# AlessioSam/LADiff

Hardware: AMD Instinct MI355X
Metric: motions/sec (196-frame, 50-step DDIM, bs128) (higher is better)
Workload: dtype f16x3+f32; 1 GPU; headline:ddim50_cfg7.5_b128_f196_c263_humanml3d; prompts_per_gpu=128, global_batch=128, frames=196, scheduler=ddim, denoising_steps=50, parallelism=dp1, loop=persistent pipeline kernel (16-row blocks x 86)

## Files before the change

### ladiff_amd/build.py

```python
import os
import subprocess
import sys
from concurrent.futures import ThreadPoolExecutor

HERE = os.path.dirname(os.path.abspath(__file__))
CSRC = os.path.join(HERE, "csrc")
OBJ = os.path.join(HERE, "csrc", "build")
LIB = os.path.join(HERE, "libladiff_hip.so")
SOURCES = ["gemm.hip", "gemm_big.hip", "gemm_kr.hip", "gemm_rowln.hip", "rowops.hip", "attention.hip", "qkv_attn.hip", "systolic.hip", "linear_ca.hip", "dec_cross.hip", "dec_mlp.hip", "dec_qkv_attn.hip", "feats2joints.hip", "denoiser.hip", "decoder.hip", "encoder.hip", "clip.hip", "evaluator.hip", "api.hip"]
FLAGS = ["--offload-arch=gfx950", "-O3", "-std=c++17", "-fPIC", "-fvisibility=hidden", "-Wall", "-Wno-unused-function"]


def _hipcc():
    for c in (os.environ.get("HIPCC"), "/opt/rocm/bin/hipcc", "hipcc"):
        if c and (os.path.isabs(c) and os.path.exists(c) or not os.path.isabs(c)):
            return c
    raise RuntimeError("hipcc not found")


def _stale(target, deps):
    if not os.path.exists(target):
        return True
    t = os.path.getmtime(target)
    return any(os.path.getmtime(d) > t for d in deps)


def stamps_lib(level=1):
    return LIB.replace(".so", "_stamps.so" if int(level) == 1 else f"_stamps{int(level)}.so")


def diag_lib():
    return LIB.replace(".so", "_diag.so")


def build(force=False, verbose=False, stamps=False, tag=None, defines=(), only=None):
    obj, lib, flags = OBJ, LIB, list(FLAGS)
    if tag:
        obj, lib = OBJ + "_" + tag, LIB.replace(".so", f"_{tag}.so")
        flags += ["-D" + d for d in defines]
    if stamps:
        lvl = os.environ.get("LADIFF_STAMPS_LEVEL", "1")
        obj, lib = OBJ + "_stamps" + (lvl if lvl != "1" else ""), stamps_lib(lvl)
        flags.append("-DLADIFF_STAMPS=" + lvl)
    os.makedirs(obj, exist_ok=True)
    headers = [os.path.join(CSRC, f) for f in os.listdir(CSRC) if f.endswith(".h")]
    headers += [os.path.join(os.path.dirname(HERE), "include", h) for h in ("ladiff_hip.h", "ladiff_hip_debug.h")]
    hipcc = _hipcc()
    jobs = []
    objdir = {src: (obj if only is None or src in only else OBJ) for src in SOURCES}
    for src in SOURCES:
        s = os.path.join(CSRC, src)
        o = os.path.join(objdir[src], src.replace(".hip", ".o"))
        if objdir[src] == obj and (force or _stale(o, [s] + headers)):
            jobs.append([hipcc, *flags, "-c", s, "-o", o])

    def run(cmd):
        if verbose:
            print(" ".join(cmd), flush=True)
        r = subprocess.run(cmd, capture_output=True, text=True)
        if r.returncode != 0:
            raise RuntimeError(f"hipcc failed: {' '.join(cmd)}\n{r.stdout}\n{r.stderr}")
        return r.stderr
# ... 27 lines not shown
```

### ladiff_amd/csrc/api.hip

```cpp
#include <algorithm>
#include <cstdlib>
#include <atomic>
#include <cstdio>
#include <cstdlib>
#include <cstring>
#include <vector>

#include "model.h"
#include "../../include/ladiff_hip_debug.h"

using namespace ladiff;

namespace {

inline hipStream_t S(ladiff_stream_t s) { return reinterpret_cast<hipStream_t>(s); }

template <class W>
bool load_weights(W& dst, const float* const* ptrs) {
    constexpr int n = sizeof(W) / sizeof(const float*);
    if (ptrs == nullptr) return false;
    for (int i = 0; i < n; ++i)
        if (ptrs[i] == nullptr) return false;
    std::memcpy(&dst, ptrs, sizeof(W));
    return true;
// ... 307 lines not shown
    int mr16 = 1, nb16 = 0, mr32 = 2, nb32 = 0;
    std::vector<unsigned char> p16, p32;
    if (!cfg) {
        sys_pack_blocks(B, T, 1, h_counts, masked, false, plan, plan_mr, plan_nb);
        return;
    }
    sys_pack_blocks(B, T, 2, h_counts, masked, true, p32, &mr32, &nb32);
    int want = loop_mode == 2 ? 1 : (loop_mode == 3 ? 2 : 0);
    if (want != 2) sys_pack_blocks(B, T, 1, h_counts, masked, true, p16, &mr16, &nb16);
    if (want == 0) {
        const double c16 = f16x3 ? 2.45 : 5.05, c32 = f16x3 ? 5.3 : 12.1, lat16 = f16x3 ? 172.0 : 310.0, lat32 = f16x3 ? 282.0 : 525.0;
        const double e16 = mr16 == 1 ? std::max(lat16, nb16 * c16) : 1e30, e32 = std::max(lat32, nb32 * c32);
        want = e16 < e32 ? 1 : 2;
    }
    if (want == 1 && mr16 == 1) { plan.swap(p16); *plan_mr = 1; *plan_nb = nb16; }
    else { plan.swap(p32); *plan_mr = 2; *plan_nb = nb32; }
}

extern "C" {

int ladiff_reverse_plan(int B, int T, const int32_t* h_counts, int masked, int loop_mode, int f16x3, int cfg, int* rows_per_block, int* n_blocks) {
    LADIFF_CHECK_ARG(B >= 1 && T >= 1 && T <= LADIFF_MAX_LATENTS && loop_mode >= 1 && loop_mode <= 3 && rows_per_block && n_blocks);
    if (!cfg && masked && h_counts == nullptr) return LADIFF_ERR_UNSUPPORTED;
    std::vector<unsigned char> plan;
    int mr = 2, nb = 0;
    choose_plan(B, T, h_counts, masked != 0, loop_mode, f16x3 != 0, plan, &mr, &nb, cfg != 0);
    *rows_per_block = 16 * mr; *n_blocks = nb;
    return 0;
}

int ladiff_debug_set_stage_waves(int waves_per_simd) {
    LADIFF_CHECK_ARG(waves_per_simd == 1 || waves_per_simd == 2);
    g_waves16 = waves_per_simd;
    return 0;
}

int ladiff_debug_set_handoff(int tagged) {
    LADIFF_CHECK_ARG(tagged == 0 || tagged == 1);
    g_handoff = tagged;
    return 0;
}

int ladiff_debug_set_mlp_variant(int v) {
#ifdef LADIFF_STAMPS
    LADIFF_CHECK_ARG((v >= 0 && v <= 3) || (v >= 11 && v <= 17) || (v >= 21 && v <= 26));
#else
    LADIFF_CHECK_ARG(v >= 0 && v <= 3);
#endif
    g_mlp_variant = v;
    return 0;
}

int ladiff_debug_set_decoder_fusion(int on) {
    LADIFF_CHECK_ARG(on >= 0 && on <= 126 && (on & 3) != 3 && (on & 48) != 48);
    g_dec_out_cross = (on & 64) ? 0 : 1;
    g_dec_fused_mlp = on & 3;
    g_dec_small_rows_path = (on & 4) ? 0 : 1;
    g_dec_final_split = (on & 8) ? 0 : 1;
    g_dec_fused_attn = (on & 16) ? 0 : (on & 32) ? 2 : 1;
    return 0;
}

int ladiff_debug_set_stage_plan(int v) {
    LADIFF_CHECK_ARG(v >= 0 && v <= 1);
    g_stage_plan = v;
    return 0;
}

int ladiff_debug_set_poll_pause(int mask, int len) {
    LADIFF_CHECK_ARG(mask >= 0 && mask <= 255 && len >= 0 && len <= 64);
    g_poll_pause = mask | (len << 8);
    return 0;
}

int ladiff_debug_set_pacing(int eighths, int mask) {
    if (eighths == -1) { g_pace = -1; return 0; }
    LADIFF_CHECK_ARG(eighths >= 0 && eighths <= 8 && mask >= 0 && mask <= 255);
    g_pace = eighths | (mask << 8);
    return 0;
}

int ladiff_debug_set_stage_delay(int mask, int len) {
    LADIFF_CHECK_ARG(mask >= -1 && mask <= 255 && len >= 0 && len <= 64);
    g_stage_delay = mask < 0 ? -1 : (mask | (len << 8));
    return 0;
}

int ladiff_debug_set_loop_thresholds(int look_ahead_from, int small_upto) {
    LADIFF_CHECK_ARG(look_ahead_from >= -1 && small_upto >= -1);
    g_look_ahead_from = look_ahead_from;
    g_small_upto = small_upto;
    return 0;
}

int ladiff_debug_set_graph_epoch_rule(int on) {
    LADIFF_CHECK_ARG(on == 0 || on == 1);
    g_graph_epoch_rule = on;
    return 0;
}

int ladiff_debug_graph_instantiations(void) { return g_graph_instantiations.load(); }

int ladiff_debug_set_xcd_local(int on) {
    LADIFF_CHECK_ARG(on >= 0 && on <= 2);
    g_xcd_local = on;
    return 0;
}
// ... 351 lines not shown
    (void)C;
    return dec_ws_floats(B, (size_t)B * F, T) * sizeof(float);
}

int ladiff_vae_decode(const float* const* w, const float* const* w_split, const float* z, const int32_t* lengths,
                      const int32_t* counts, int B, int F, int T, int C, float* feats, void* ws, size_t ws_bytes,
                      ladiff_stream_t stream) {
    DecoderW W, WS;
    LADIFF_CHECK_ARG(load_weights(W, w) && z && lengths && feats && ws && B >= 0);
    if (w_split != nullptr) LADIFF_CHECK_ARG(load_weights(WS, w_split));
    return vae_decode(W, w_split ? &WS : nullptr, z, lengths, counts, nullptr, 0, B, F, T, C, feats, (float*)ws, ws_bytes / sizeof(float),
                      S(stream));
}

namespace {
struct DecodeGraph {
    hipGraphExec_t exec = nullptr;
    hipStream_t cap = nullptr;
    int cap_dev = -1;
    const void* key_ptrs[7] = {nullptr};
    uint64_t epoch = 0;
    int key_ints[6] = {0};
    uint64_t key_hash = 0, key_gen = 0;
};
}

int ladiff_decoder_graph_create(void** graph) {
    LADIFF_CHECK_ARG(graph);
    *graph = new DecodeGraph();
    return 0;
}
int ladiff_decoder_graph_destroy(void* graph) {
    DecodeGraph* g = reinterpret_cast<DecodeGraph*>(graph);
    if (g == nullptr) return 0;
    (void)hipDeviceSynchronize();
    if (g->exec) (void)hipGraphExecDestroy(g->exec);
    if (g->cap) (void)hipStreamDestroy(g->cap);
    delete g;
    return 0;
}

int ladiff_vae_decode_graphed(void* graph, const float* const* w, const float* const* w_split, uint64_t weights_generation, const float* z,
                              const int32_t* lengths, const int32_t* counts, const int32_t* row_off, int total_rows, int B, int F, int T,
                              int C, float* feats, void* ws, size_t ws_bytes, ladiff_stream_t stream) {
    DecodeGraph* dg = reinterpret_cast<DecodeGraph*>(graph);
    DecoderW W, WS;
    LADIFF_CHECK_ARG(dg && load_weights(W, w) && z && lengths && feats && ws && B >= 0 && stream != nullptr);
    if (w_split != nullptr) LADIFF_CHECK_ARG(load_weights(WS, w_split));
    hipStream_t s = S(stream);
    const void* kp[7] = {z, lengths, counts, row_off, feats, ws, stream};
    const int ki[6] = {B, F, T, C, total_rows, w_split ? 1 : 0};
    uint64_t h = hash_ptrs(w, DEC_NPARAMS, 1469598103934665603ull);
    if (w_split) h = hash_ptrs(w_split, DEC_NPARAMS, h ^ 0x9e3779b97f4a7c15ull);
    h ^= (uint64_t)(g_dec_fused_mlp + 4 * g_dec_small_rows_path + 8 * g_dec_final_split + 16 * g_mlp_variant + 4096 * g_dec_fused_attn) * 0x100000001b3ull;
    const bool same = dg->exec && std::memcmp(kp, dg->key_ptrs, sizeof(kp)) == 0 && std::memcmp(ki, dg->key_ints, sizeof(ki)) == 0 &&
                      h == dg->key_hash && weights_generation == dg->key_gen &&
                      (dg->epoch == g_graph_epoch.load() || g_graph_epoch_rule.load() == 0);
    if (!same) {
        if (dg->exec) { LADIFF_HIP(hipStreamSynchronize(s)); (void)hipGraphExecDestroy(dg->exec); dg->exec = nullptr; }
        LADIFF_TRY(dec_mlp_prepare());
        LADIFF_TRY(dec_qkv_attn_prepare());
        LADIFF_TRY(dec_cross_prepare());
        hipGraph_t gr = nullptr;
        LADIFF_TRY(capture_stream(&dg->cap, &dg->cap_dev));
        const hipStream_t cs = dg->cap;
        LADIFF_HIP(hipStreamBeginCapture(cs, hipStreamCaptureModeThreadLocal));
        int rc = 0;
        if (row_off != nullptr) {
            rc = launch_zero_fill(feats, (size_t)B * F * C, cs);
        }
        if (rc == 0) rc = vae_decode(W, w_split ? &WS : nullptr, z, lengths, counts, row_off, total_rows, B, F, T, C, feats, (float*)ws,
                                     ws_bytes / sizeof(float), cs);
        const hipError_t ec = hipStreamEndCapture(cs, &gr);
        if (rc != 0) { if (gr) (void)hipGraphDestroy(gr); return rc; }
        LADIFF_HIP(ec);
        const hipError_t ei = hipGraphInstantiate(&dg->exec, gr, nullptr, nullptr, 0);
        ++g_graph_instantiations;
        (void)hipGraphDestroy(gr);
        LADIFF_HIP(ei);
        std::memcpy(dg->key_ptrs, kp, sizeof(kp));
        std::memcpy(dg->key_ints, ki, sizeof(ki));
        dg->key_hash = h; dg->key_gen = weights_generation;
        dg->epoch = ++g_graph_epoch;
    }
    LADIFF_HIP(hipGraphLaunch(dg->exec, s));
    return 0;
}

int ladiff_vae_decode_ragged(const float* const* w, const float* const* w_split, const float* z, const int32_t* lengths,
                             const int32_t* counts, const int32_t* row_off, int total_rows, int B, int F, int T, int C, float* feats,
                             void* ws, size_t ws_bytes, ladiff_stream_t stream) {
    DecoderW W, WS;
    LADIFF_CHECK_ARG(load_weights(W, w) && z && lengths && row_off && feats && ws && B >= 0 && total_rows >= 0);
    if (w_split != nullptr) LADIFF_CHECK_ARG(load_weights(WS, w_split));
    LADIFF_HIP(hipMemsetAsync(feats, 0, (size_t)B * F * C * sizeof(float), S(stream)));
    return vae_decode(W, w_split ? &WS : nullptr, z, lengths, counts, row_off, total_rows, B, F, T, C, feats, (float*)ws,
                      ws_bytes / sizeof(float), S(stream));
}

}
```

### ladiff_amd/csrc/decoder.hip

```cpp
#include "model.h"
#ifdef LADIFF_STAMPS
#include <cstdlib>
#endif

namespace ladiff {

#ifdef LADIFF_STAMPS
#define DEC_CUT() do { if (dec_cut >= 0 && ++dec_launched >= dec_cut) return 0; } while (0)
#else
#define DEC_CUT() do { } while (0)
#endif

constexpr int DEC_SMALL_ROWS = 4096;
std::atomic<int> g_dec_out_cross{1};
std::atomic<int> g_dec_fused_attn{1};
std::atomic<int> g_dec_final_split{1};
std::atomic<int> g_dec_small_rows_path{1};
std::atomic<int> g_dec_fused_mlp{1};

static GemmArgs lin(const float* A, int lda, const float* W, const float* bias, float* Y, int ldy, int M, int N, int K,
                    int act = ACT_NONE) {
    GemmArgs g;
    g.A = A; g.lda = lda; g.W = W; g.ldw = K; g.bias = bias; g.Y = Y; g.ldy = ldy; g.M = M; g.N = N; g.K = K; g.act = act;
    return g;
}

size_t dec_ws_floats(int B, size_t rows, int T) {
    return rows * (16 * D + 3 * D + D + FF) + (rows + 63) / 64 * 64 + (size_t)NL * ((size_t)T * B * 2 * D + dec_cross_ws_floats(B, T)) +
           (size_t)LADIFF_MAX_FRAMES * (2 * D + 3 * D);
}

int vae_decode(const DecoderW& w, const DecoderW* wsp, const float* z, const int32_t* lengths, const int32_t* counts,
               const int32_t* row_off, int R, int B, int F, int T, int C, float* feats, float* ws, size_t ws_floats, hipStream_t s) {
    if (F < 1 || F > LADIFF_MAX_FRAMES || T < 1 || T > LADIFF_MAX_LATENTS || C < 1) return LADIFF_ERR_SHAPE;
    const bool ragged = row_off != nullptr;
    if (ragged && (R < 0 || (size_t)R > (size_t)B * F)) return LADIFF_ERR_SHAPE;
    const int M = ragged ? R : B * F;
    if (ws_floats < dec_ws_floats(B, (size_t)M, T)) return LADIFF_ERR_WORKSPACE;
    if (M == 0) return 0;
#ifdef LADIFF_STAMPS
    const char* dec_cut_env = getenv("LADIFF_DEC_CUT");
    const int dec_cut = dec_cut_env ? atoi(dec_cut_env) : -1;
    int dec_launched = 0;
    if (dec_cut == 0) return 0;
#endif
    const bool sp = wsp != nullptr;
    const size_t MD = (size_t)M * D;
    float* P[4]; float* SK[NSKIP]; float* Ps[4]; float* SKs[NSKIP];
    float* p = ws;
    for (int i = 0; i < 4; ++i) { P[i] = p; p += MD; }
    for (int i = 0; i < NSKIP; ++i) { SK[i] = p; p += MD; }
    for (int i = 0; i < 4; ++i) { Ps[i] = sp ? p : nullptr; p += MD; }
    for (int i = 0; i < NSKIP; ++i) { SKs[i] = sp ? p : nullptr; p += MD; }
    float* qkv = p; p += 3 * MD;
    float* att = p; p += MD;
    float* hid = p; p += (size_t)M * FF;
    float* kv = p; p += (size_t)NL * T * B * 2 * D;
    float* guws = p; p += (size_t)NL * dec_cross_ws_floats(B, T);
    int32_t* row_out = reinterpret_cast<int32_t*>(p); p += ((size_t)M + 63) / 64 * 64;
    float* pex = p; p += (size_t)LADIFF_MAX_FRAMES * D;
    float* pexs = p; p += (size_t)LADIFF_MAX_FRAMES * D;
    float* qkv0 = p;
    const size_t kv_l = (size_t)T * B * 2 * D, gu_l = dec_cross_ws_floats(B, T);

    {
        GemmArgs g[NL];
        DecCrossPrepBatch pb;
        for (int l = 0; l < NL; ++l) {
            const DecLayerW& L = w.layer[l];
            g[l] = lin(z, D, L.cross_attn.in_w + (size_t)D * D, L.cross_attn.in_b + D, kv + l * kv_l, 2 * D, T * B, 2 * D, D);
// ... 26 lines not shown
        g.split = 1;
        LADIFF_TRY(launch_gemm(g, s));
        if (n2)
            return launch_reduce_rows(dst, 1, M, nullptr, nullptr, RED_LN, n1.g, n1.b, nullptr, 0, nullptr, nullptr, 1, 1, 0,
                                      0, dst, dsts, s, nullptr, n2->g, n2->b);
        return launch_reduce_rows(dst, 1, M, nullptr, nullptr, RED_LN, n1.g, n1.b, nullptr, 0, nullptr, nullptr, 1, 1, 0, 0,
                                  dst, dsts, s);
    };

    if (ragged) { LADIFF_TRY(launch_broadcast_pe_ragged(w.query_pe, row_off, B, F, F, P[0], Ps[0], row_out, s)); DEC_CUT(); }
    else { LADIFF_TRY(launch_broadcast_pe(w.query_pe, B, F, P[0], Ps[0], s)); DEC_CUT(); }
    const float* cur = P[0]; const float* curs = Ps[0];
    for (int l = 0; l < NL; ++l) {
        const DecLayerW& L = w.layer[l];
        const DecLayerW& Ls = sp ? wsp->layer[l] : w.layer[l];
        const bool is_in = l < NSKIP, is_out = l > NSKIP, last = l == NL - 1;
        if (is_out) {
            const LinearW& sk = w.skip[l - NSKIP - 1];
            if (small) {
                RowLnArgs g;
                g.A = curs; g.lda = D; g.A2 = SKs[NL - 1 - l]; g.lda2 = D; g.K1 = D; g.W = wsp->skip[l - NSKIP - 1].w; g.ldw = 2 * D; g.bias = sk.b;
                g.Y = P[3]; g.Ys = Ps[3]; g.ldy = D; g.M = M; g.K = 2 * D;
                LADIFF_TRY(launch_gemm_rowln(g, s)); DEC_CUT();
            } else {
            GemmArgs g = lin(sp ? curs : cur, D, sp ? wsp->skip[l - NSKIP - 1].w : sk.w, sk.b, P[3], D, M, D, 2 * D);
            g.A2 = sp ? SKs[NL - 1 - l] : SK[NL - 1 - l]; g.lda2 = D; g.K1 = D;
            g.split = sp ? 1 : 0; g.Ys = Ps[3];
            LADIFF_TRY(launch_gemm(g, s)); DEC_CUT();
            }
            cur = P[3]; curs = Ps[3];
        }
        const bool shared = l == 0;
        if (shared) {
            LADIFF_TRY(launch_broadcast_pe(w.query_pe, 1, F, pex, sp ? pexs : nullptr, s)); DEC_CUT();
            if (small) { LADIFF_TRY(krs(pexs, D, Ls.self_attn.in_w, L.self_attn.in_b, qkv0, nullptr, 3 * D, 3 * D, ACT_NONE, nullptr, F)); DEC_CUT(); }
            else {
            GemmArgs g = lin(sp ? pexs : pex, D, Ls.self_attn.in_w, L.self_attn.in_b, qkv0, 3 * D, F, 3 * D, D);
            g.split = sp ? 1 : 0;
            LADIFF_TRY(launch_gemm(g, s)); DEC_CUT();
            }
        } else if (fused_attn) {
        } else if (small) {
            LADIFF_TRY(krs(curs, D, Ls.self_attn.in_w, L.self_attn.in_b, qkv, nullptr, 3 * D, 3 * D, ACT_NONE, nullptr, M)); DEC_CUT();
        } else {
            GemmArgs g = lin(sp ? curs : cur, D, Ls.self_attn.in_w, L.self_attn.in_b, qkv, 3 * D, M, 3 * D, D);
            g.split = sp ? 1 : 0;
            LADIFF_TRY(launch_gemm(g, s)); DEC_CUT();
        }
        const float* qkv_l = shared ? qkv0 : qkv;
        if (fused_attn && !shared) { LADIFF_TRY(launch_dec_qkv_attn(curs, Ls.self_attn.in_w, L.self_attn.in_b, lengths, row_off, att, B, F, 1, s)); DEC_CUT(); }
        else if (sp) { LADIFF_TRY(launch_self_attention_split(qkv_l, lengths, nullptr, att, B, F, H, 0, 1, s, row_off, shared)); DEC_CUT(); }
        else { LADIFF_TRY(launch_decoder_self_attention(qkv_l, lengths, nullptr, att, B, F, 0, s, row_off, shared)); DEC_CUT(); }
        const NormW* n1_late = nullptr;
        if (sp && !small && g_dec_out_cross) {
            LADIFF_TRY(launch_decoder_out_cross(att, cur, Ls.self_attn.out_w, L.self_attn.out_b, L.norm1.g, L.norm1.b, L.cross_attn.out_b,
                                                L.norm2.g, L.norm2.b, counts, B, F, T, guws + l * gu_l, P[2], Ps[2], s, row_off)); DEC_CUT();
        } else {
        if (sp) {
            if (small) { LADIFF_TRY(krs(att, D, Ls.self_attn.out_w, L.self_attn.out_b, P[1], nullptr, D, D, ACT_NONE, cur, M)); DEC_CUT(); }
            else {
            GemmArgs g = lin(att, D, Ls.self_attn.out_w, L.self_attn.out_b, P[1], D, M, D, D);
            g.res = cur; g.ldres = D; g.split = 1;
            LADIFF_TRY(launch_gemm(g, s)); DEC_CUT();
            }
            n1_late = &L.norm1;
        } else {
            LADIFF_TRY(gemm_ln(att, D, L.self_attn.out_w, Ls.self_attn.out_w, L.self_attn.out_b, cur, L.norm1, nullptr, P[1], nullptr)); DEC_CUT();
        }
        LADIFF_TRY(launch_decoder_cross_apply(P[1], L.cross_attn.out_b, L.norm2.g, L.norm2.b, counts, B, F, T, guws + l * gu_l, P[2],
                                              Ps[2], s, row_off, n1_late ? n1_late->g : nullptr, n1_late ? n1_late->b : nullptr)); DEC_CUT();
        }
        float* dst = is_in ? SK[l] : P[0];
        float* dsts = is_in ? SKs[l] : Ps[0];
        if (sp && g_dec_fused_mlp && (M >= dec_mlp_min_rows() || g_dec_fused_mlp == 2)) {
            LADIFF_TRY(launch_dec_mlp(Ps[2], P[2], Ls.lin1.w, L.lin1.b, Ls.lin2.w, L.lin2.b, L.norm3.g, L.norm3.b,
                                      last ? w.norm.g : nullptr, last ? w.norm.b : nullptr, dst, dsts, M, s)); DEC_CUT();
        } else if (small) {
            LADIFF_TRY(krs(Ps[2], D, Ls.lin1.w, L.lin1.b, nullptr, hid, FF, FF, ACT_GELU, nullptr, M)); DEC_CUT();
            LADIFF_TRY(krs(hid, FF, Ls.lin2.w, nullptr, qkv, nullptr, D, D, ACT_NONE, nullptr, M)); DEC_CUT();
            LADIFF_TRY(launch_reduce_rows(qkv, 4, M, L.lin2.b, P[2], RED_LN, L.norm3.g, L.norm3.b, nullptr, 0, nullptr, nullptr, 1, 1, 0, 0,
                                          dst, dsts, s, nullptr, last ? w.norm.g : nullptr, last ? w.norm.b : nullptr));
        } else {
            GemmArgs g = lin(sp ? Ps[2] : P[2], D, Ls.lin1.w, L.lin1.b, sp ? nullptr : hid, FF, M, FF, D, ACT_GELU);
            g.split = sp ? 1 : 0; if (sp) g.Ys = hid;
            LADIFF_TRY(launch_gemm(g, s)); DEC_CUT();
            LADIFF_TRY(gemm_ln(hid, FF, L.lin2.w, Ls.lin2.w, L.lin2.b, P[2], L.norm3, last ? &w.norm : nullptr, dst, dsts)); DEC_CUT();
        }
        cur = dst; curs = dsts;
    }
    if (sp && M >= DEC_SMALL_ROWS && g_dec_final_split) {
        const int Np = (C + 127) / 128 * 128;
        if ((size_t)Np > (size_t)FF || (size_t)Np * (D + 1) > 3 * MD) return LADIFF_ERR_SHAPE;
        float* wpad = qkv; float* bpad = qkv + (size_t)Np * D;
        LADIFF_TRY(launch_pad_rows(wsp->final_layer.w, w.final_layer.b, wpad, bpad, C, Np, s)); DEC_CUT();
        GemmArgs g = lin(curs, D, wpad, bpad, hid, Np, M, Np, D);
        g.split = 1;
        LADIFF_TRY(launch_gemm(g, s)); DEC_CUT();
        return launch_scatter_feats(hid, Np, C, M, F, ragged ? nullptr : lengths, ragged ? row_out : nullptr, feats, s);
    }
    GemmArgs g = lin(cur, D, w.final_layer.w, w.final_layer.b, feats, C, M, C, D);
    if (ragged) g.row_map = row_out;
    else { g.row_len = lengths; g.rows_per_item = F; }
    return launch_gemm(g, s);
}

}
```

### ladiff_amd/csrc/model.h

```cpp
#pragma once
#include <atomic>
#include "gemm.h"
#include "gemm_kr.h"
#include "kernels.h"
#include "weights.h"

namespace ladiff {

constexpr int DEN_OFF_CA_MOD = 0;
constexpr int DEN_OFF_FFN_MOD = 2 * D;
constexpr int DEN_OFF_TIME_KV = 4 * D;
constexpr int DEN_LAYER_STRIDE = 6 * D;
constexpr int DEN_STEP_STRIDE = NL * DEN_LAYER_STRIDE;

size_t den_tables_floats(int n_steps);
size_t den_text_cache_floats(int B2, int n_steps, int ntxt = 1);
size_t den_text_ws_floats(int B2, int n_steps, int ntxt = 1);
size_t den_forward_ws_floats(int B2, int T);
int denoiser_time_tables(const DenoiserW& w, const float* sinus, int n, float* tables, float* ws, size_t ws_floats, hipStream_t s);
int denoiser_text_cache(const DenoiserW& w, const float* text, int B2, const float* tables, int n_steps, float* cache,
                        float* ws, size_t ws_floats, hipStream_t s, int ntxt = 1);
int denoiser_forward(const DenoiserW& w, const DenoiserW* w_split, const float* tables, const int32_t* d_step,
                     const float* cache, int n_steps, const float* sample, int Bs, int dup, int T, const int32_t* counts, float* eps, float* ws,
                     size_t ws_floats, hipStream_t s, int b_lo = 0, int b_n = -1, int loop_mode = 0, int ntxt = 1,
                     const int32_t* d_base = nullptr);
const float* den_cache_tkv(const float* cache, int B2, int ntxt);
const float* den_cache_ctab(const float* cache, int B2, int ntxt);
int denoiser_text_static(const DenoiserW& w, const float* text, int B2, float* cache, float* ws, size_t ws_floats, hipStream_t s);
int denoiser_ctab(const DenoiserW& w, const float* tables_lo, int n, float* cache, int B2, float* u, size_t u_floats, hipStream_t s,
                  const DenoiserW* w_split = nullptr);
int linear_cross_attention(const DenoiserW& w, int layer, const float* x, const float* xf, const float* emb, const int32_t* counts,
                           int B, int T, int N, float* out, float* ws, size_t ws_floats, hipStream_t s);
size_t linear_cross_attention_ws_floats(int B, int T, int N);
void den_loop_io(float* ws, int rows, float** x, float** xs);

extern std::atomic<int> g_dec_fused_mlp;
extern std::atomic<int> g_dec_small_rows_path;
extern std::atomic<int> g_dec_final_split;
extern std::atomic<int> g_dec_out_cross;
extern std::atomic<int> g_stage_plan;
extern std::atomic<int> g_poll_pause;
extern std::atomic<int> g_stage_delay;
extern std::atomic<int> g_pace;
extern std::atomic<int> g_look_ahead_from, g_small_upto;
extern std::atomic<int> g_dec_fused_attn;
extern std::atomic<int> g_mlp_variant;
int dec_mlp_prepare();
int dec_qkv_attn_prepare();
int dec_cross_prepare();
int dec_mlp_min_rows();
size_t dec_ws_floats(int B, size_t rows, int T);
int vae_decode(const DecoderW& w, const DecoderW* w_split, const float* z, const int32_t* lengths, const int32_t* counts,
               const int32_t* row_off, int R, int B, int F, int T, int C, float* feats, float* ws, size_t ws_floats, hipStream_t s);

int launch_dec_mlp(const float* xs, const float* x, const float* w1, const float* b1, const float* w2, const float* b2, const float* g3,
                   const float* be3, const float* g4, const float* be4, float* y, float* ys, int M, hipStream_t s);

size_t enc_ws_floats(int B, int F, int T, int C);
int vae_encode(const EncoderW& w, const EncoderW* w_split, const float* features, const int32_t* lengths,
               const int32_t* counts, const float* eps, int B, int F, int T, int C, float* mu, float* sd, float* latent, float* ws,
               size_t ws_floats, hipStream_t s);

#ifdef LADIFF_STAMPS
extern unsigned long long* g_sys_stamps;
extern int g_sys_probe;
#endif
size_t sys_ws_floats(int B, int T);
bool sys_supported(int B, int T, int cfg, bool split);
extern std::atomic<int> g_waves16;
extern std::atomic<int> g_handoff;
int sys_reset_status(float* ws, hipStream_t s);
extern std::atomic<int> g_xcd_local;
void sys_pack_blocks(int B, int T, int want_mr, const int32_t* h_counts, bool masked, bool cfg, std::vector<unsigned char>& out, int* mr, int* nb);
int sys_build_stages(const DenoiserW& W, const DenoiserW& WS, float* ws, int MR, int NB, std::vector<unsigned char>& host);
size_t sys_blocks_offset_floats(int MR, int NB);
size_t sys_status_offset_floats(int B, int T);
int launch_systolic_loop(const DenoiserW& W, float* ws, const float* tables, const float* tkv, const float* ctab, int n_ctab,
                         const float* coef, const float* noise, float* lat, const int32_t* counts, float gscale, int B, int T,
                         int step_lo, int n, int fp32, int MR, int NB, hipStream_t s, int cfg = 1, int fault_wg = -1,
                         unsigned long long timeout_ticks = 0, const NoiseGen& gen = NoiseGen{0u, 0u, 0u, 0});

int launch_qkv_attention(const float* x, const float* w, const float* bias, const float* text_kv, const float* tables,
                         int kv_off, int step_stride, const int32_t* d_step, const int32_t* counts, int Bs, int b_off,
                         int b_n, int T, float* out, hipStream_t s);

size_t clip_ws_floats(int B, int L);
size_t clip_ws_floats_rows(int B, int total_rows);
int clip_text_encode(const ClipW& w, const ClipW* w_split, int n_layers, int vocab, const int64_t* ids, int B, int S, int L,
                     float* out, float* ws, size_t ws_floats, hipStream_t s, const int32_t* seq_len = nullptr,
                     const int32_t* row_off = nullptr, const int32_t* row_seq = nullptr, int total_rows = 0);

const std::vector<std::string>& t2m_move_param_names();
const std::vector<std::string>& t2m_motion_param_names();
const std::vector<std::string>& t2m_text_param_names();
size_t t2m_move_ws_floats(int B, int F, int Cin);
size_t t2m_motion_ws_floats(int B, int T);
size_t t2m_text_ws_floats(int B, int L);
int t2m_movement_encode(const float* const* w, const float* feats, int ld, int B, int F, int Cin, float* out, float* ws,
                        size_t ws_floats, hipStream_t s);
int t2m_motion_encode(const float* const* w, const float* mov, const int32_t* m_lens, int B, int T, float* out, float* ws,
                      size_t ws_floats, hipStream_t s);
int t2m_text_encode(const float* const* w, const float* word_embs, const float* pos_onehot, const int32_t* cap_lens, int B, int L,
                    float* out, float* ws, size_t ws_floats, hipStream_t s);

}
```

Baseline: 11290 motions/s.

## Fuse decoder self-attn out-proj, cross-attn apply and MLP into one tail kernel

Adds a dec_tail kernel that, per 128-row block, runs the self-attention output projection with residual and LayerNorm, the cross-attention against a prepacked latent image, and the full FFN with GELU and final LayerNorms, all in registers. Weights stream through an 8-stage LDS ring via global_load_lds DMA. This replaces the separate out_cross and dec_mlp launches and their intermediate global round-trips in each decoder layer. In exchange it needs a large LDS footprint and a complex hand-scheduled pipeline. It only covers the VAE decode stage, not the denoising loop.

```diff
diff --git a/ladiff_amd/build.py b/ladiff_amd/build.py
--- a/ladiff_amd/build.py
+++ b/ladiff_amd/build.py
@@ -7,7 +7,7 @@
 CSRC = os.path.join(HERE, "csrc")
 OBJ = os.path.join(HERE, "csrc", "build")
 LIB = os.path.join(HERE, "libladiff_hip.so")
-SOURCES = ["gemm.hip", "gemm_big.hip", "gemm_kr.hip", "gemm_rowln.hip", "rowops.hip", "attention.hip", "qkv_attn.hip", "systolic.hip", "linear_ca.hip", "dec_cross.hip", "dec_mlp.hip", "dec_qkv_attn.hip", "feats2joints.hip", "denoiser.hip", "decoder.hip", "encoder.hip", "clip.hip", "evaluator.hip", "api.hip"]
+SOURCES = ["gemm.hip", "gemm_big.hip", "gemm_kr.hip", "gemm_rowln.hip", "rowops.hip", "attention.hip", "qkv_attn.hip", "systolic.hip", "linear_ca.hip", "dec_cross.hip", "dec_mlp.hip", "dec_tail.hip", "dec_qkv_attn.hip", "feats2joints.hip", "denoiser.hip", "decoder.hip", "encoder.hip", "clip.hip", "evaluator.hip", "api.hip"]
 FLAGS = ["--offload-arch=gfx950", "-O3", "-std=c++17", "-fPIC", "-fvisibility=hidden", "-Wall", "-Wno-unused-function"]
 
 
diff --git a/ladiff_amd/csrc/api.hip b/ladiff_amd/csrc/api.hip
--- a/ladiff_amd/csrc/api.hip
+++ b/ladiff_amd/csrc/api.hip
@@ -383,7 +383,8 @@
 }
 
 int ladiff_debug_set_decoder_fusion(int on) {
-    LADIFF_CHECK_ARG(on >= 0 && on <= 126 && (on & 3) != 3 && (on & 48) != 48);
+    LADIFF_CHECK_ARG(on >= 0 && on <= 254 && (on & 3) != 3 && (on & 48) != 48);
+    g_dec_tail = (on & 128) ? 0 : 1;
     g_dec_out_cross = (on & 64) ? 0 : 1;
     g_dec_fused_mlp = on & 3;
     g_dec_small_rows_path = (on & 4) ? 0 : 1;
@@ -841,7 +842,7 @@
     const int ki[6] = {B, F, T, C, total_rows, w_split ? 1 : 0};
     uint64_t h = hash_ptrs(w, DEC_NPARAMS, 1469598103934665603ull);
     if (w_split) h = hash_ptrs(w_split, DEC_NPARAMS, h ^ 0x9e3779b97f4a7c15ull);
-    h ^= (uint64_t)(g_dec_fused_mlp + 4 * g_dec_small_rows_path + 8 * g_dec_final_split + 16 * g_mlp_variant + 4096 * g_dec_fused_attn) * 0x100000001b3ull;
+    h ^= (uint64_t)(g_dec_fused_mlp + 4 * g_dec_small_rows_path + 8 * g_dec_final_split + 16 * g_mlp_variant + 4096 * g_dec_fused_attn + 65536 * g_dec_out_cross + 131072 * g_dec_tail) * 0x100000001b3ull;
     const bool same = dg->exec && std::memcmp(kp, dg->key_ptrs, sizeof(kp)) == 0 && std::memcmp(ki, dg->key_ints, sizeof(ki)) == 0 &&
                       h == dg->key_hash && weights_generation == dg->key_gen &&
                       (dg->epoch == g_graph_epoch.load() || g_graph_epoch_rule.load() == 0);
@@ -850,6 +851,7 @@
         LADIFF_TRY(dec_mlp_prepare());
         LADIFF_TRY(dec_qkv_attn_prepare());
         LADIFF_TRY(dec_cross_prepare());
+        LADIFF_TRY(dec_tail_prepare());
         hipGraph_t gr = nullptr;
         LADIFF_TRY(capture_stream(&dg->cap, &dg->cap_dev));
         const hipStream_t cs = dg->cap;
diff --git a/ladiff_amd/csrc/dec_tail.hip b/ladiff_amd/csrc/dec_tail.hip
--- /dev/null
+++ b/ladiff_amd/csrc/dec_tail.hip
@@ -0,0 +1,385 @@
+#include <mutex>
+#include "model.h"
+#include "tile_mma.h"
+
+namespace ladiff {
+
+namespace {
+
+constexpr int TL_NW = 8;
+constexpr int TL_ROWS = 16 * TL_NW;
+constexpr int TL_NS = 8;
+constexpr int TL_GRP = 4;
+constexpr int TL_STAGE = 16384;
+constexpr int TL_FRONT = 20;
+constexpr int TL_IMG = 4 * TL_STAGE / 4;
+constexpr int TL_NV = 11;
+constexpr int TL_LDS = TL_NS * TL_STAGE + FF * 4 + TL_NV * D * 4 + 32 * 4;
+
+typedef unsigned u32x4_t __attribute__((ext_vector_type(4)));
+
+struct TailArgs {
+    const float* att;
+    const float* x0;
+    const float* wo;
+    const float* img;
+    const float* cc;
+    const float* w1; const float* b1; const float* w2;
+    const float* vec[TL_NV];
+    const int32_t* counts; const int32_t* row_off;
+    float* y; float* ys;
+    int F, T, rows_per_wg;
+};
+
+__host__ __device__ __forceinline__ int pi_row(int p) { const int j = p >> 4, n = p & 15; return 32 * (j >> 1) + 8 * (n >> 2) + 4 * (j & 1) + (n & 3); }
+
+__device__ __forceinline__ void wait_vm0() { asm volatile("s_waitcnt vmcnt(0)" ::: "memory"); }
+template <int OFF>
+__device__ __forceinline__ void fetch16(u32x4_t& v, unsigned addr) {
+    asm volatile("ds_read_b128 %0, %1 offset:%2" : "=v"(v) : "v"(addr), "n"(OFF) : "memory");
+}
+__device__ __forceinline__ void wait_lgkm0(u32x4_t& a, u32x4_t& b, u32x4_t& c, u32x4_t& d) {
+    asm volatile("s_waitcnt lgkmcnt(0)" : "+v"(a), "+v"(b), "+v"(c), "+v"(d));
+}
+__device__ __forceinline__ s16x8 as_s16(const u32x4_t v) { return __builtin_bit_cast(s16x8, v); }
+__device__ __forceinline__ int acc_col(int jj, int fk) { return 32 * (jj >> 1) + 8 * fk + 4 * (jj & 1); }
+
+__device__ __forceinline__ void acc_ln(f32x4 (&v)[16], const float* gp, const float* bp, int fk) {
+    float s = 0.f;
+#pragma unroll
+    for (int jj = 0; jj < 16; ++jj) s += (v[jj][0] + v[jj][1]) + (v[jj][2] + v[jj][3]);
+    s += __shfl_xor(s, 16, 64); s += __shfl_xor(s, 32, 64);
+    const float mean = s * (1.f / 256.f);
+    float q = 0.f;
+#pragma unroll
+    for (int jj = 0; jj < 16; ++jj)
+#pragma unroll
+        for (int e = 0; e < 4; ++e) { v[jj][e] -= mean; q = fmaf(v[jj][e], v[jj][e], q); }
+    q += __shfl_xor(q, 16, 64); q += __shfl_xor(q, 32, 64);
+    const float rstd = rsqrtf(q * (1.f / 256.f) + LN_EPS);
+#pragma unroll
+    for (int jj = 0; jj < 16; ++jj) {
+        const int col = acc_col(jj, fk);
+        const f32x4 ga = ld4(gp + col), be = ld4(bp + col);
+#pragma unroll
+        for (int e = 0; e < 4; ++e) v[jj][e] = v[jj][e] * rstd * ga[e] + be[e];
+    }
+}
+
+}
+
+__global__ __launch_bounds__(1024) void dec_tail_image_kernel(const float* __restrict__ gu, int T, float* __restrict__ img) {
+    const int b = blockIdx.x, st = blockIdx.y, p = threadIdx.x >> 3, ps = threadIdx.x & 7;
+    const int ls = ps ^ ((p >> 1) & 7), k0 = 8 * (ls & 3);
+    const float* gub = gu + (size_t)b * H * T * 2 * D;
+    f32x4 a = {0.f, 0.f, 0.f, 0.f}, c = a;
+    if (st < 2) {
+        const int j = p >> 4, n = p & 15, hj = 8 * (n >> 2) + 4 * st + (n & 3), h = hj >> 3, t = hj & 7;
+        if (t < T) { const float* g = gub + (size_t)(h * T + t) * 2 * D + 32 * j + k0; a = ld4(g); c = ld4(g + 4); }
+    } else {
+        const int n = 128 * (st - 2) + pi_row(p);
+#pragma unroll
+        for (int e = 0; e < 8; ++e) {
+            const int kk = k0 + e, h = kk >> 3, t = kk & 7;
+            const float u = t < T ? gub[((size_t)(h * T + t) * 2 + 1) * D + n] : 0.f;
+            if (e < 4) a[e] = u; else c[e - 4] = u;
+        }
+    }
+    s16x8 hi, lo;
+    split8(a, c, hi, lo);
+    *reinterpret_cast<s16x8*>(img + (size_t)b * TL_IMG + st * (TL_STAGE / 4) + p * 32 + ps * 4) = ls < 4 ? hi : lo;
+}
+
+__global__ __launch_bounds__(64 * TL_NW, 2) void dec_tail_kernel(const TailArgs p) {
+    constexpr int NW = TL_NW, NT = 64 * NW, PPW = 16 / NW, H2 = PPW / 2;
+    extern __shared__ __attribute__((aligned(1024))) char lds[];
+    float* const b1s = reinterpret_cast<float*>(lds + TL_NS * TL_STAGE);
+    float* const prm = b1s + FF;
+    float* const cs = prm + TL_NV * D;
+    const int b = blockIdx.x, tid = threadIdx.x, lane = tid & 63;
+    const int wave = __builtin_amdgcn_readfirstlane(tid >> 6);
+    const int frow = lane & 15, fk = lane >> 4;
+    int F = p.F;
+    size_t row0 = (size_t)b * F;
+    if (p.row_off != nullptr) { row0 = p.row_off[b]; F = p.row_off[b + 1] - p.row_off[b]; }
+    const int f0 = blockIdx.y * p.rows_per_wg;
+    const int f1 = f0 + p.rows_per_wg < F ? f0 + p.rows_per_wg : F;
+    if (f0 >= f1) return;
+    const int T = p.T;
+    int nv = p.counts != nullptr ? p.counts[b] : T;
+    nv = nv > T ? T : nv;
+    const int ft = f0 + 16 * wave;
+    const bool act = ft < f1;
+    const size_t myrow = row0 + (ft + frow < f1 ? ft + frow : f1 - 1);
+
+    s16x8 xh[8], xl[8];
+    {
+        const char* xr = reinterpret_cast<const char*>(p.att) + myrow * 1024 + fk * 16;
+#pragma unroll
+        for (int s = 0; s < 8; ++s) {
+            xh[s] = *reinterpret_cast<const s16x8*>(xr + (s >> 1) * 256 + (s & 1) * 64);
+            xl[s] = *reinterpret_cast<const s16x8*>(xr + (s >> 1) * 256 + (s & 1) * 64 + 128);
+        }
+    }
+    f32x4 oacc[16], hacc[8], sacc[2][2];
+#pragma unroll
+    for (int jj = 0; jj < 16; ++jj) {
+        const int col = acc_col(jj, fk);
+        const f32x4 r = ld4(p.x0 + myrow * D + col), bo = ld4(p.vec[5] + col);
+#pragma unroll
+        for (int e = 0; e < 4; ++e) oacc[jj][e] = r[e] + bo[e];
+    }
+    for (int i = tid; i < FF / 4; i += NT) st4(b1s + 4 * i, ld4(p.b1 + 4 * i));
+    for (int i = tid; i < TL_NV * D / 4; i += NT) {
+        const float* src = p.vec[i / (D / 4)];
+        if (src != nullptr) st4(prm + 4 * i, ld4(src + 4 * (i % (D / 4))));
+    }
+    if (tid < 32) { const int h = tid >> 3, t = tid & 7; cs[tid] = t < T ? p.cc[((size_t)b * H + h) * T + t] : 0.f; }
+
+    const int csl = (lane & 7) ^ ((lane >> 4) & 3) ^ (4 * (wave & 1));
+    const int koff = (csl < 4 ? csl * 4 : 32 + (csl - 4) * 4);
+    int src[PPW];
+#pragma unroll
+    for (int i = 0; i < PPW; ++i) src[i] = pi_row(8 * (wave + NW * i) + (lane >> 3));
+    char* const dma_dst = lds + (8 * wave) * 128;
+    const int limg = (8 * wave + (lane >> 3)) * 32 + (lane & 7) * 4;
+    int loff[PPW], loff2[PPW];
+#pragma unroll
+    for (int i = 0; i < PPW; ++i) { loff[i] = src[i] * D + koff; loff2[i] = src[i] * FF + koff; }
+    auto at = [&](const float* base, int lo) __attribute__((always_inline)) { asm volatile("" : "+v"(lo)); return base + lo; };
+    auto dma = [&](const float* s0, int slot, int i) __attribute__((always_inline)) {
+        __builtin_amdgcn_global_load_lds(s0, (__attribute__((address_space(3))) void*)(dma_dst + slot * TL_STAGE + 8 * NW * i * 128), 16, 0, 0);
+    };
+    auto issue = [&](auto gc, int hs, auto ic) __attribute__((always_inline)) {
+        constexpr int g = decltype(gc)::value, i = decltype(ic)::value, slot = g % TL_NS;
+        if constexpr (g < 16) {
+            constexpr int k = g >> 1;
+            dma(at(p.wo + 128 * (g & 1) * D + (k >> 1) * 64 + (k & 1) * 16, loff[i]), slot, i);
+        } else if constexpr (g < TL_FRONT) {
+            dma(at(p.img + (size_t)b * TL_IMG + (g - 16) * (TL_STAGE / 4) + 8 * NW * i * 32, limg), slot, i);
+        } else {
+            constexpr int u = (g - TL_FRONT) % 16;
+            const int hsv = hs & 7;
+            if constexpr (u < 8) dma(at(p.w1 + 128 * hsv * D + (u >> 1) * 64 + (u & 1) * 16, loff[i]), slot, i);
+            else {
+                constexpr int v = u - 8, c = v >> 1;
+                dma(at(p.w2 + 128 * (v & 1) * FF + (2 * hsv + (c >> 1)) * 64 + (c & 1) * 16, loff2[i]), slot, i);
+            }
+        }
+    };
+
+    const int sw = (frow >> 1) & 7;
+    const unsigned rd_hi = lds_addr(lds) + frow * 128 + ((fk ^ sw) << 4);
+    const unsigned rd_lo = lds_addr(lds) + frow * 128 + (((4 + fk) ^ sw) << 4);
+    const unsigned rd_hi2 = rd_hi + 4 * TL_STAGE, rd_lo2 = rd_lo + 4 * TL_STAGE;
+    u32x4_t wt[4][2];
+    auto fetch_tile = [&](auto slotc, auto jc) __attribute__((always_inline)) {
+        constexpr int slot = decltype(slotc)::value, j = decltype(jc)::value, so = (slot & 3) * TL_STAGE;
+        fetch16<so + j * 2048>(wt[j & 3][0], slot < 4 ? rd_hi : rd_hi2);
+        fetch16<so + j * 2048>(wt[j & 3][1], slot < 4 ? rd_lo : rd_lo2);
+    };
+    auto stage_mma = [&](auto slotc, auto&& prod, auto&& between, auto&& next) __attribute__((always_inline)) {
+        constexpr int slot = decltype(slotc)::value;
+        static_for<8>([&](auto jc) {
+            constexpr int j = decltype(jc)::value, cur = j & 3;
+            next(jc);
+            {
+                asm volatile("s_waitcnt lgkmcnt(4)" : "+v"(wt[cur][0]), "+v"(wt[cur][1]));
+                __builtin_amdgcn_sched_barrier(0);
+                prod(jc, IntC<0>{}, as_s16(wt[cur][0]));
+                __builtin_amdgcn_sched_barrier(0);
+                if constexpr (j + 3 < 8) fetch_tile(slotc, IntC<j + 3>{});
+                else fetch_tile(IntC<(slot + 1) % TL_NS>{}, IntC<j + 3 - 8>{});
+                __builtin_amdgcn_sched_barrier(0);
+                prod(jc, IntC<1>{}, as_s16(wt[cur][1]));
+                prod(jc, IntC<2>{}, as_s16(wt[cur][0]));
+            }
+            __builtin_amdgcn_sched_barrier(0);
+            if constexpr (j & 1) between(IntC<j / 2>{});
+        });
+    };
+    auto onto = [&](f32x4 (&acc)[16], auto j0c, const s16x8& bh, const s16x8& bl) __attribute__((always_inline)) {
+        return [&acc, &bh, &bl](auto jc, auto prodc, s16x8 w) __attribute__((always_inline)) {
+            constexpr int j = decltype(jc)::value + decltype(j0c)::value, pr = decltype(prodc)::value;
+            acc[j] = MFMA16_S16(w, pr == 0 ? bl : bh, acc[j], 0, 0, 0);
+        };
+    };
+
+    auto drain = [&]() __attribute__((always_inline)) {
+        wait_lgkm0(wt[0][0], wt[0][1], wt[1][0], wt[1][1]);
+        wait_lgkm0(wt[2][0], wt[2][1], wt[3][0], wt[3][1]);
+    };
+    auto landed = [&]() __attribute__((always_inline)) { wait_vm0(); __builtin_amdgcn_s_barrier(); };
+    auto run = [&](auto gc, int hs, auto&& prod) __attribute__((always_inline)) {
+        constexpr int g = decltype(gc)::value, slot = g % TL_NS, r = g % TL_GRP;
+        auto batch = [&](auto aheadc, auto halfc) __attribute__((always_inline)) {
+            constexpr int ahead = decltype(aheadc)::value, half = decltype(halfc)::value;
+            constexpr int gt = g + ahead;
+            constexpr int gtc = gt < TL_FRONT + 16 ? gt : gt - 16;
+            const int hs_t = gt < TL_FRONT + 16 ? hs : hs + 1;
+            static_for<H2>([&](auto ic) { issue(IntC<gtc>{}, hs_t, IntC<H2 * half + decltype(ic)::value>{}); });
+        };
+        auto between = [&](auto gc2) __attribute__((always_inline)) {
+            constexpr int gg = decltype(gc2)::value;
+            if constexpr (r == 3 && gg >= 2) batch(IntC<5>{}, IntC<gg - 2>{});
+            else if constexpr (r == 0 && gg < 2) batch(IntC<5>{}, IntC<gg>{});
+            else if constexpr (r == 0 && gg >= 2) batch(IntC<6>{}, IntC<gg - 2>{});
+            else if constexpr (r == 1 && gg < 2) batch(IntC<6>{}, IntC<gg>{});
+        };
+        auto next = [&](auto jc) __attribute__((always_inline)) {
+            constexpr int j = decltype(jc)::value;
+            if constexpr (r == 3 && j == 5) landed();
+            else if constexpr (r == 0 && j == 5) __builtin_amdgcn_s_barrier();
+        };
+        stage_mma(IntC<slot>{}, prod, between, next);
+    };
+
+    static_for<TL_GRP>([&](auto uc) { static_for<PPW>([&](auto ic) { issue(IntC<decltype(uc)::value>{}, 0, ic); }); });
+    __syncthreads();
+    landed();
+    static_for<PPW>([&](auto ic) { issue(IntC<TL_GRP>{}, 0, ic); });
+    static_for<3>([&](auto jc) { fetch_tile(IntC<0>{}, jc); });
+
+    static_for<16>([&](auto gc) {
+        constexpr int g = decltype(gc)::value;
+        run(gc, 0, onto(oacc, IntC<8 * (g & 1)>{}, xh[g >> 1], xl[g >> 1]));
+    });
+    drain();
+    acc_ln(oacc, prm + 6 * D, prm + 7 * D, fk);
+#pragma unroll
+    for (int c = 0; c < 8; ++c) split8(oacc[2 * c], oacc[2 * c + 1], xh[c], xl[c]);
+#pragma unroll
+    for (int s = 0; s < 2; ++s) { sacc[s][0] = f32x4{0.f, 0.f, 0.f, 0.f}; sacc[s][1] = sacc[s][0]; }
+    static_for<2>([&](auto sc) {
+        constexpr int s = decltype(sc)::value;
+        run(IntC<16 + s>{}, 0, [&](auto jc, auto prodc, s16x8 w) __attribute__((always_inline)) {
+            constexpr int j = decltype(jc)::value, pr = decltype(prodc)::value;
+            sacc[s][j & 1] = MFMA16_S16(w, pr == 0 ? xl[j] : xh[j], sacc[s][j & 1], 0, 0, 0);
+        });
+    });
+    drain();
+    s16x8 ph, pl;
+    {
+        float sv[8];
+#pragma unroll
+        for (int t = 0; t < 8; ++t) sv[t] = (sacc[t >> 2][0][t & 3] + sacc[t >> 2][1][t & 3]) + cs[8 * fk + t];
+        float m = -INFINITY, l = 0.f;
+#pragma unroll
+        for (int t = 0; t < 8; ++t) m = t < nv ? fmaxf(m, sv[t]) : m;
+#pragma unroll
+        for (int t = 0; t < 8; ++t) { sv[t] = t < nv ? __builtin_amdgcn_exp2f((sv[t] - m) * 1.4426950408889634f) : 0.f; l += sv[t]; }
+        const float inv = 1.f / l;
+        f32x4 pa, pb;
+#pragma unroll
+        for (int e = 0; e < 4; ++e) { pa[e] = sv[e] * inv; pb[e] = sv[4 + e] * inv; }
+        split8(pa, pb, ph, pl);
+    }
+#pragma unroll
+    for (int jj = 0; jj < 16; ++jj) {
+        const f32x4 bc = ld4(prm + 8 * D + acc_col(jj, fk));
+#pragma unroll
+        for (int e = 0; e < 4; ++e) oacc[jj][e] = ((float)xh[jj >> 1][4 * (jj & 1) + e] + (float)xl[jj >> 1][4 * (jj & 1) + e]) + bc[e];
+    }
+    static_for<2>([&](auto sc) { run(IntC<18 + decltype(sc)::value>{}, 0, onto(oacc, IntC<8 * decltype(sc)::value>{}, ph, pl)); });
+    drain();
+    acc_ln(oacc, prm + 9 * D, prm + 10 * D, fk);
+#pragma unroll
+    for (int c = 0; c < 8; ++c) split8(oacc[2 * c], oacc[2 * c + 1], xh[c], xl[c]);
+#pragma unroll
+    for (int jj = 0; jj < 16; ++jj) {
+        const f32x4 b2 = ld4(prm + acc_col(jj, fk));
+#pragma unroll
+        for (int e = 0; e < 4; ++e) oacc[jj][e] += b2[e];
+    }
+
+    s16x8 hh[4], hl[4];
+#pragma unroll 1
+    for (int hs = 0; hs < 8; ++hs) {
+        static_for<16>([&](auto uc) {
+            constexpr int u = decltype(uc)::value;
+            if constexpr (u < 8) {
+                if constexpr (u == 0) {
+#pragma unroll
+                    for (int j = 0; j < 8; ++j) hacc[j] = f32x4{0.f, 0.f, 0.f, 0.f};
+                }
+                run(IntC<TL_FRONT + u>{}, hs, [&](auto jc, auto prodc, s16x8 w) __attribute__((always_inline)) {
+                    constexpr int j = decltype(jc)::value, pr = decltype(prodc)::value;
+                    hacc[j] = MFMA16_S16(w, pr == 0 ? xl[u] : xh[u], hacc[j], 0, 0, 0);
+                });
+            } else {
+                constexpr int v = u - 8, c = v >> 1, nh = v & 1;
+                if constexpr (nh == 0) {
+                    const f32x4 ba = ld4(b1s + 128 * hs + 32 * c + 8 * fk), bb = ld4(b1s + 128 * hs + 32 * c + 8 * fk + 4);
+                    f32x4 va, vb;
+#pragma unroll
+                    for (int e = 0; e < 4; ++e) { va[e] = gelu_erf(hacc[2 * c][e] + ba[e]); vb[e] = gelu_erf(hacc[2 * c + 1][e] + bb[e]); }
+                    split8(va, vb, hh[c], hl[c]);
+                }
+                run(IntC<TL_FRONT + u>{}, hs, onto(oacc, IntC<8 * nh>{}, hh[c], hl[c]));
+            }
+        });
+    }
+    wait_vm0();
+    wait_lgkm0(wt[0][0], wt[0][1], wt[1][0], wt[1][1]);
+    wait_lgkm0(wt[2][0], wt[2][1], wt[3][0], wt[3][1]);
+
+    __syncthreads();
+    acc_ln(oacc, prm + 1 * D, prm + 2 * D, fk);
+    if (p.vec[3] != nullptr) acc_ln(oacc, prm + 3 * D, prm + 4 * D, fk);
+    if (!act) return;
+    char* const stg = lds + wave * 16384;
+#pragma unroll
+    for (int jj = 0; jj < 16; ++jj) {
+        const int ch = 8 * (jj >> 1) + 2 * fk + (jj & 1);
+        *reinterpret_cast<f32x4*>(stg + frow * 1024 + ((ch ^ frow) << 4)) = oacc[jj];
+    }
+#pragma unroll
+    for (int r = 0; r < 16; ++r) {
+        const f32x4 o = *reinterpret_cast<const f32x4*>(stg + r * 1024 + ((lane ^ r) << 4));
+        if (ft + r < f1) {
+            const size_t row = row0 + ft + r;
+            if (p.y != nullptr) st4(p.y + row * D + 4 * lane, o);
+            if (p.ys != nullptr) store_split4(p.ys + row * D, 4 * lane, o);
+        }
+    }
+}
+
+int dec_tail_prepare() {
+    static std::mutex mu;
+    static bool attr_set[64] = {};
+    int dev = 0;
+    LADIFF_HIP(hipGetDevice(&dev));
+    if (dev < 0 || dev >= 64) return LADIFF_ERR_ARG;
+    std::lock_guard<std::mutex> lock(mu);
+    if (!attr_set[dev]) {
+        LADIFF_HIP(hipFuncSetAttribute(reinterpret_cast<const void*>(dec_tail_kernel), hipFuncAttributeMaxDynamicSharedMemorySize, TL_LDS));
+        attr_set[dev] = true;
+    }
+    return 0;
+}
+
+size_t dec_tail_img_floats(int B) { return (size_t)B * TL_IMG; }
+
+int launch_dec_tail(const DecTailArgs& a, hipStream_t s) {
+    if (a.B == 0 || a.F == 0) return 0;
+    if (a.T < 1 || a.T > LADIFF_MAX_LATENTS) return LADIFF_ERR_SHAPE;
+    LADIFF_TRY(dec_tail_prepare());
+    hipLaunchKernelGGL(dec_tail_image_kernel, dim3(a.B, 4), dim3(1024), 0, s, a.gu, a.T, a.img);
+    LADIFF_LAUNCH_CHECK();
+    int chunks = (256 + a.B - 1) / a.B;
+    if (chunks > (a.F + 15) / 16) chunks = (a.F + 15) / 16;
+    if (chunks < (a.F + TL_ROWS - 1) / TL_ROWS) chunks = (a.F + TL_ROWS - 1) / TL_ROWS;
+    const int rows_per_wg = (a.F + chunks - 1) / chunks;
+    chunks = (a.F + rows_per_wg - 1) / rows_per_wg;
+    TailArgs t;
+    t.att = a.att; t.x0 = a.x0; t.wo = a.wo; t.img = a.img; t.cc = a.gu + (size_t)a.B * H * a.T * 2 * D;
+    t.w1 = a.w1; t.b1 = a.b1; t.w2 = a.w2;
+    const float* v[TL_NV] = {a.b2, a.g3, a.be3, a.g4, a.be4, a.bo, a.g1, a.be1, a.bo_c, a.g2, a.be2};
+    for (int i = 0; i < TL_NV; ++i) t.vec[i] = v[i];
+    t.counts = a.counts; t.row_off = a.row_off; t.y = a.y; t.ys = a.ys; t.F = a.F; t.T = a.T; t.rows_per_wg = rows_per_wg;
+    hipLaunchKernelGGL(dec_tail_kernel, dim3(a.B, chunks), dim3(64 * TL_NW), TL_LDS, s, t);
+    LADIFF_LAUNCH_CHECK();
+    return 0;
+}
+
+}
diff --git a/ladiff_amd/csrc/decoder.hip b/ladiff_amd/csrc/decoder.hip
--- a/ladiff_amd/csrc/decoder.hip
+++ b/ladiff_amd/csrc/decoder.hip
@@ -16,6 +16,7 @@
 std::atomic<int> g_dec_fused_attn{1};
 std::atomic<int> g_dec_final_split{1};
 std::atomic<int> g_dec_small_rows_path{1};
+std::atomic<int> g_dec_tail{1};
 std::atomic<int> g_dec_fused_mlp{1};
 
 static GemmArgs lin(const float* A, int lda, const float* W, const float* bias, float* Y, int ldy, int M, int N, int K,
@@ -148,6 +149,21 @@
         else if (sp) { LADIFF_TRY(launch_self_attention_split(qkv_l, lengths, nullptr, att, B, F, H, 0, 1, s, row_off, shared)); DEC_CUT(); }
         else { LADIFF_TRY(launch_decoder_self_attention(qkv_l, lengths, nullptr, att, B, F, 0, s, row_off, shared)); DEC_CUT(); }
         const NormW* n1_late = nullptr;
+        float* dst = is_in ? SK[l] : P[0];
+        float* dsts = is_in ? SKs[l] : Ps[0];
+        const bool tail = sp && !small && g_dec_out_cross && g_dec_tail && g_dec_fused_mlp && (M >= dec_mlp_min_rows() || g_dec_fused_mlp == 2) &&
+                          (g_mlp_variant == 0 || g_mlp_variant == 1) && dec_tail_img_floats(B) <= (size_t)M * FF;
+        if (tail) {
+            DecTailArgs ta;
+            ta.att = att; ta.x0 = cur; ta.wo = Ls.self_attn.out_w; ta.bo = L.self_attn.out_b; ta.g1 = L.norm1.g; ta.be1 = L.norm1.b;
+            ta.gu = guws + l * gu_l; ta.bo_c = L.cross_attn.out_b; ta.g2 = L.norm2.g; ta.be2 = L.norm2.b;
+            ta.w1 = Ls.lin1.w; ta.b1 = L.lin1.b; ta.w2 = Ls.lin2.w; ta.b2 = L.lin2.b; ta.g3 = L.norm3.g; ta.be3 = L.norm3.b;
+            ta.g4 = last ? w.norm.g : nullptr; ta.be4 = last ? w.norm.b : nullptr;
+            ta.counts = counts; ta.row_off = row_off; ta.img = hid; ta.y = dst; ta.ys = dsts; ta.B = B; ta.F = F; ta.T = T;
+            LADIFF_TRY(launch_dec_tail(ta, s)); DEC_CUT();
+            cur = dst; curs = dsts;
+            continue;
+        }
         if (sp && !small && g_dec_out_cross) {
             LADIFF_TRY(launch_decoder_out_cross(att, cur, Ls.self_attn.out_w, L.self_attn.out_b, L.norm1.g, L.norm1.b, L.cross_attn.out_b,
                                                 L.norm2.g, L.norm2.b, counts, B, F, T, guws + l * gu_l, P[2], Ps[2], s, row_off)); DEC_CUT();
@@ -166,8 +182,6 @@
         LADIFF_TRY(launch_decoder_cross_apply(P[1], L.cross_attn.out_b, L.norm2.g, L.norm2.b, counts, B, F, T, guws + l * gu_l, P[2],
                                               Ps[2], s, row_off, n1_late ? n1_late->g : nullptr, n1_late ? n1_late->b : nullptr)); DEC_CUT();
         }
-        float* dst = is_in ? SK[l] : P[0];
-        float* dsts = is_in ? SKs[l] : Ps[0];
         if (sp && g_dec_fused_mlp && (M >= dec_mlp_min_rows() || g_dec_fused_mlp == 2)) {
             LADIFF_TRY(launch_dec_mlp(Ps[2], P[2], Ls.lin1.w, L.lin1.b, Ls.lin2.w, L.lin2.b, L.norm3.g, L.norm3.b,
                                       last ? w.norm.g : nullptr, last ? w.norm.b : nullptr, dst, dsts, M, s)); DEC_CUT();
diff --git a/ladiff_amd/csrc/model.h b/ladiff_amd/csrc/model.h
--- a/ladiff_amd/csrc/model.h
+++ b/ladiff_amd/csrc/model.h
@@ -56,6 +56,19 @@
 int launch_dec_mlp(const float* xs, const float* x, const float* w1, const float* b1, const float* w2, const float* b2, const float* g3,
                    const float* be3, const float* g4, const float* be4, float* y, float* ys, int M, hipStream_t s);
 
+struct DecTailArgs {
+    const float* att; const float* x0; const float* wo; const float* bo; const float* g1; const float* be1;
+    const float* gu; const float* bo_c; const float* g2; const float* be2;
+    const float* w1; const float* b1; const float* w2; const float* b2; const float* g3; const float* be3; const float* g4; const float* be4;
+    const int32_t* counts; const int32_t* row_off;
+    float* img; float* y; float* ys;
+    int B, F, T;
+};
+extern std::atomic<int> g_dec_tail;
+int dec_tail_prepare();
+size_t dec_tail_img_floats(int B);
+int launch_dec_tail(const DecTailArgs& a, hipStream_t s);
+
 size_t enc_ws_floats(int B, int F, int T, int C);
 int vae_encode(const EncoderW& w, const EncoderW* w_split, const float* features, const int32_t* lengths,
                const int32_t* counts, const float* eps, int B, int F, int T, int C, float* mu, float* sd, float* latent, float* ws,
```

Result: no change. 11300 motions/s, median of 6 (+0.1%).
